# Autonomous-Drone-Racing-Lab/Efficient-Path-Planner

Measured on AMD Instinct MI355X. Metric: validity checks/sec + full plan ms/track, 1/2/4/8 MI355X vs CPU ref, higher is better.
Workload: dtype f64; 1 GPU; C2: 1 track, 8 gates, 64 OBBs, 1,048,576 sampled states per step; obbs=64, can_pass_gate=False, parallelism=replicas x1 (independent samplers), process_group=solo, launch=hip graph of the K steps

## Files before the change

### efficient-path-planner_amd/csrc/epp_internal.h

```cpp
#pragma once
#include <math.h>
#include <stdint.h>

#include <mutex>
#include <shared_mutex>
#include <string>
#include <vector>

#include <hip/hip_runtime_api.h>

#include "epp.h"

namespace epp {
epp_status generate_trajectory_into(const double* wp, int32_t n_wp, const double* times, double v_max,
                                    double a_max, double dt, double t0, const double v0[3], const double a0[3],
                                    double* (*alloc)(void*, int64_t), void* ctx, int64_t* n_rows);
struct FusedCheck {
    const epp_world* world;
    const double* xyz;
    int64_t n;
    double min_distance;
    uint8_t* valid;
};
epp_status check_and_generate_into(const FusedCheck* chk, const double* wp, int32_t n_wp, const double* times,
// ... 22 lines not shown
                                  const int64_t* rows_n, int32_t cap, int32_t k, int32_t can_pass_gate,
                                  uint8_t* valid, uint16_t* out16, int32_t target, int64_t* count, void* stream,
                                  const MotionMask* marks = nullptr);
bool knn_motions_rows_supported(const epp_world* world);

struct PlanSeg {
    uint64_t seed;
    double s[3], g[3];
    double bound;
    double gbound;
    double glo[3], ghi[3];
    double h;
    int64_t row_off;
    int64_t need_off;
    int32_t cap;
    int32_t need_cap;
};
enum : int { kPbRows = 1, kPbPerSeg = 3 };
struct PlanBatchLayout {
    int32_t S = 0, k = 0, ns_log = 0, nbc = 0, cap_total = 0, nctr = 0;
    int64_t ns = 0, NS = 0, need_cap = 0;
    size_t o_seg = 0, o_ctr = 0, o_xyz = 0, o_valid = 0, o_nodes = 0, o_cstat = 0, o_kws = 0, kws_stride = 0,
           o_query = 0, o_ids32 = 0, o_rows32 = 0, o_rows16 = 0, o_ev = 0, o_mark = 0, o_map = 0, o_nstat = 0,
           o_need = 0, dev_bytes = 0;
    size_t h_seg = 0, h_hdr = 0, h_slot = 0, h_rows = 0, h_need = 0, h_done = 0, host_bytes = 0;
    int32_t done_n = 0;
};
PlanBatchLayout plan_batch_layout(int32_t S, int64_t ns, int32_t k, PlanSeg* segs);
void plan_batch_trace_print();
epp_status plan_batch_launch(const epp_world* world, int32_t can_pass_gate, const double lo[3], const double hi[3],
                             const PlanBatchLayout& L, void* dev, void* host, uint32_t seq, void* stream);
}

namespace epp {

enum Field : int {
    F_LOX = 0, F_LOY, F_LOZ, F_HIX, F_HIY, F_HIZ,
    F_CX, F_CY, F_CZ,
    F_COS, F_SIN,
    F_HX, F_HY, F_HZ,
    EPP_NF
};

constexpr int kRecDoubles = 17;
constexpr int R_META = 16;

constexpr int kPtDoubles = 16;
constexpr int P_TX = F_HX, P_TY = F_HY, P_TZ = F_HZ;
#if defined(__HIPCC__)
__host__ __device__
#endif
constexpr uint32_t pt_chunk_off(uint32_t i, uint32_t c) { return (i << 7) + ((c ^ ((i >> 1) & 7u)) << 4); }
constexpr uint32_t kIdFill = 0x8000u;

constexpr size_t kListMaxLen = 4095;
constexpr size_t kStageBudget = 64 * 1024;

constexpr uint32_t META_FILLING = 1u;
constexpr uint32_t META_GATE = 2u;
constexpr int kMaxGridAxis = 255;

struct WorldView {
    const unsigned char* blob;
    uint32_t blob_bytes;
    int32_t n_obb;
    int32_t n_pad;
    int32_t nx, ny, nz;
    uint32_t front_bytes;
    uint32_t off_cell_mask;
    uint32_t off_cell_start;
    uint32_t off_cell_obb;
    uint32_t off_meta;
    uint32_t off_soa;
    double gx0, gy0, gz0;
    double gx1, gy1, gz1;
    double icx, icy, icz;
    float ofx, ofy, ofz;
    float i4x, i4y, i4z;
    float limx, limy, limz;
    float fmaxx, fmaxy, fmaxz;
    double r_gate, r_obst;
    uint32_t off_aos;
    uint32_t off_pt;
    uint32_t off_lists;
    uint32_t off_ids;
    uint32_t id_mask;
    uint32_t n_lists;
    uint32_t off_bitmap;
    uint32_t bm_words;
    uint32_t off_cls8;
    uint32_t cls8_bytes;
    int32_t bnx, bny, bnz;
    float bofx, bofy, bofz;
    float bix, biy, biz;
    uint32_t off_slab;
    int32_t slab_n;
    int32_t slab_log;
    int32_t slab_w;
    int32_t tile_n;
    uint32_t tile_words;
    float sofx, sofy, sofz;
    float six, siy, siz;
};

constexpr int kSlabMaxWords = 32;
constexpr size_t kSlabBudget = 40 * 1024;
constexpr size_t kSlabBudgetMax = 64 * 1024;
constexpr size_t kMotionsLdsFree = 150 * 1024 - 16 * (256 * 4 + 64);
#if defined(__HIPCC__)
__host__ __device__
#endif
constexpr int slab_row_stride(int w) { return (w & 1) ? w : w + 1; }

#if defined(__HIPCC__)
__host__ __device__
#endif
inline int slab_axis(double p, float off, float inv, int S) {
    float f = fmaf((float)p, inv, off);
    f = fminf(fmaxf(f, 0.0f), (float)(S - 1));
    return (int)f;
}

#if defined(__HIPCC__)
__host__ __device__
#endif
inline int bm_axis(double p, float off, float inv) {
    float f = fmaf((float)p, inv, off);
    f = fminf(fmaxf(f, -1.0f), 16777216.0f);
    return (int)f;
}

struct HostWorld {
    WorldView view{};
    std::vector<epp_obb> obbs;
    struct RecReader {
        hipStream_t stream;
        hipEvent_t ev;
        bool pending;
    };
    double* h_recs = nullptr;
    double* rec_buf[2] = {nullptr, nullptr};
    size_t rec_cap[2] = {0, 0};
    int rec_slot = 0;
    std::vector<RecReader> rec_readers[2];
    bool index_stale = false;
    std::mutex mu;
    std::shared_mutex index_mu;
    WorldView dev_view{};
    double r_gate = 0, r_obst = 0;
    int device = 0;
    void* d_blob = nullptr;
    const WorldView* d_view = nullptr;
    size_t d_capacity = 0;
    void* h_stage = nullptr;
    size_t h_capacity = 0;
    hipStream_t stream = nullptr;
    uint64_t generation = 0;
    std::string blob;
    std::vector<double> aabbs;
};

#if defined(__HIPCC__)
__host__ __device__
#endif
inline float fine_coord(double p, float o, float inv4) {
    return ((float)p - o) * inv4;
}
#if defined(__HIPCC__)
__host__ __device__
#endif
inline int fine_index(float f, int n) {
    const int nf = 4 * n;
    if (!(f >= 0.0f)) return 0;
    if (f >= (float)nf) return nf - 1;
    const int c = (int)f;
    return c < nf ? c : nf - 1;
}

void set_error(const std::string& msg);

struct SmallWorld {
    const double* recs;
    int32_t n_obb;
    double r_gate, r_obst;
    int host_slot;
    std::shared_lock<std::shared_mutex> lease;
};

struct IndexLease {
    std::shared_lock<std::shared_mutex> lk;
    WorldView view{};
    const WorldView* dview = nullptr;
};
epp_status ensure_index(const epp_world* w, IndexLease* lease = nullptr);

}
```

### efficient-path-planner_amd/csrc/states_v5.hip

```cpp
#include "states_diag.h"
#include "states_kernels.h"

namespace epp {
namespace {

constexpr int kStatesPerLane = 4;

struct WaveQueue5 {
    double x[64], y[64], z[64];
    uint32_t hdr[64];
};
template <int BLOCK>
constexpr uint32_t queue5_bytes() { return (BLOCK / 64) * sizeof(WaveQueue5); }

__device__ __forceinline__ uint32_t cell_axis5(double p, float off, float inv, uint32_t nm1) {
    const float f = fmaf((float)p, inv, off);
    int i;
    asm("v_cvt_i32_f32 %0, %1" : "=v"(i) : "v"(f));
    return min((uint32_t)i, nm1);
}
__device__ __forceinline__ uint32_t mad_u24(uint32_t a, uint32_t b, uint32_t c) {
    uint32_t r;
    asm("v_mad_u32_u24 %0, %1, %2, %3" : "=v"(r) : "v"(a), "s"(b), "v"(c));
    return r;
}
__device__ __forceinline__ uint32_t lane_scatter(uint32_t target, uint32_t data) {
    return (uint32_t)__builtin_amdgcn_ds_permute((int)((target & 63u) << 2), (int)data);
}

__device__ __forceinline__ bool point_rec_hit(const unsigned char* pts, uint32_t ide, double px, double py, double pz,
                                              bool can_pass) {
    typedef double f64x2 __attribute__((ext_vector_type(2)));
    const uint32_t i = ide & (kIdFill - 1u);
    f64x2 q[7];
#pragma unroll
    for (uint32_t k = 0; k < 7; ++k) q[k] = *reinterpret_cast<const f64x2*>(pts + pt_chunk_off(i, k));
    const double lox = q[0].x, loy = q[0].y, loz = q[1].x, hix = q[1].y, hiy = q[2].x, hiz = q[2].y;
    const double cx = q[3].x, cy = q[3].y, cz = q[4].x, c = q[4].y, s = q[5].x;
    const double tx = q[5].y, ty = q[6].x, tz = q[6].y;
    const bool in = (lox < px) & (px < hix) & (loy < py) & (py < hiy) & (loz < pz) & (pz < hiz);
    const bool skip = ((ide & kIdFill) != 0u) & can_pass;
    const double dx = px - cx, dy = py - cy, dz = pz - cz;
    const double lx = c * dx + s * dy;
    const double ly = c * dy - s * dx;
    return in & !skip & (fabs(lx) <= tx) & (fabs(ly) <= ty) & (fabs(dz) <= tz);
}

__device__ __forceinline__ bool states_exact_pt(const unsigned char* sbase, uint32_t lists_off, uint32_t ids_off,
                                                double px, double py, double pz, uint32_t cls, int can_pass) {
    const uint32_t h = reinterpret_cast<const uint32_t*>(sbase + lists_off)[cls];
    const uint16_t* ids = reinterpret_cast<const uint16_t*>(sbase + ids_off) + (h >> 12);
    const uint32_t cnt = h & 4095u;
    bool hit = false;
    for (uint32_t j = 0; j < cnt; ++j) hit |= point_rec_hit(sbase, ids[j], px, py, pz, can_pass != 0);
    return hit;
}

#ifdef EPP_STATES_TL
__device__ unsigned long long g_states_tl[kTlWaves][kTlWords];
#endif

struct V5Args {
    uint32_t lists_off, ids_off;
    uint32_t cls_off, cls_nz_off;
    uint32_t nx, ny, nz;
    float ox, oy, oz, ix, iy, iz;
};

template <bool MINDIST, bool COMPACT, int BLOCK, bool PREFETCH, bool C8, int SC>
__global__ __launch_bounds__(BLOCK) __attribute__((amdgpu_waves_per_eu(BLOCK == 512 && !PREFETCH ? 5 : BLOCK / 256)))
void k_states_v5(const unsigned char* stage_src, const double* xyz,
                                                     int64_t groups, uint32_t stage_bytes, int can_pass,
                                                     int64_t n, double md, uint8_t* __restrict__ valid,
                                                     int32_t* __restrict__ compact_idx,
                                                     unsigned long long* __restrict__ n_valid, V5Args wa) {
    __shared__ WaveQueue5 queues[BLOCK / 64];
    extern __shared__ __attribute__((aligned(16))) unsigned char lds_blob[];
    const int lane = threadIdx.x & 63;
    EPP_STL(0);
    WaveQueue5* qu = &queues[threadIdx.x >> 6];
    const int64_t stride = (int64_t)gridDim.x * BLOCK;
    const int64_t gfirst = (int64_t)blockIdx.x * BLOCK;
    int64_t g = gfirst + threadIdx.x;
    constexpr int NV = 3 * kStatesPerLane;
    double va[NV], vb[NV];
    const double* xyzb = groups > 0 ? xyz : reinterpret_cast<const double*>(stage_src);
    auto load = [&](int64_t grp, double (&dst)[NV]) {
        grp = grp < groups ? grp : groups - 1;
        grp = grp < 0 ? 0 : grp;
        const double2* q = reinterpret_cast<const double2*>(xyzb) + (NV / 2) * grp;
#pragma unroll
        for (int k = 0; k < NV / 2; ++k) {
            const double2 t = q[k];
            dst[2 * k] = t.x;
            dst[2 * k + 1] = t.y;
        }
    };
    typedef unsigned int u32x4 __attribute__((ext_vector_type(4)));
    constexpr int kStageChunks = SC;
    u32x4 stg[kStageChunks];
    const uint32_t n16 = stage_bytes / 16u;
#if defined(__HIP_DEVICE_COMPILE__)
    typedef const __attribute__((address_space(1))) u32x4* gptr_stage;
    const gptr_stage ssrc = (gptr_stage)stage_src;
#else
    const u32x4* ssrc = reinterpret_cast<const u32x4*>(stage_src);
#endif
#pragma unroll
    for (int i = 0; i < kStageChunks; ++i) {
        const uint32_t o = (uint32_t)(i * BLOCK) + threadIdx.x;
        stg[i] = ssrc[o < n16 ? o : n16 - 1u];
    }
    load(g, va);
#pragma unroll
    for (int i = 0; i < kStageChunks; ++i) {
        const uint32_t o = (uint32_t)(i * BLOCK) + threadIdx.x;
        *reinterpret_cast<u32x4*>(lds_blob + 16u * (o < n16 ? o : n16)) = stg[i];
    }
    const uint32_t lists_off = wa.lists_off, ids_off = wa.ids_off;
    const unsigned char* cls_base = lds_blob + wa.cls_off;
    [[maybe_unused]] const unsigned char* cls_nz = lds_blob + wa.cls_nz_off;
    const uint32_t* hdrs = reinterpret_cast<const uint32_t*>(lds_blob + lists_off);
    const uint16_t* ids_all = reinterpret_cast<const uint16_t*>(lds_blob + ids_off);
    const float ox = wa.ox, oy = wa.oy, oz = wa.oz, ix = wa.ix, iy = wa.iy, iz = wa.iz;
    const uint32_t nx = wa.nx, ny = wa.ny, nz = wa.nz;
    __syncthreads();
    EPP_STL(1);
    auto hit_of = [&](uint32_t ide, double px, double py, double pz) -> bool {
        if constexpr (MINDIST)
            return rec_hit<true>(reinterpret_cast<const double*>(lds_blob) + (size_t)(ide & (kIdFill - 1u)) * kRecDoubles,
                                 0.0, 0.0, px, py, pz, false, md);
        else
            return point_rec_hit(lds_blob, ide, px, py, pz, can_pass != 0);
    };
    auto cell_of = [&](double px, double py, double pz) -> uint32_t {
        const uint32_t cx = cell_axis5(px, ox, ix, nx - 1), cy = cell_axis5(py, oy, iy, ny - 1),
                       cz = cell_axis5(pz, oz, iz, nz - 1);
        return mad_u24(mad_u24(cz, ny, cy), nx, cx);
    };
    auto classes_of = [&](const auto& idx, auto& c, auto& occ) {
        constexpr int N = (int)(sizeof(idx) / sizeof(idx[0]));
        if (C8) {
            uint64_t wd[N];
            uint32_t rank[N];
#pragma unroll
            for (int k = 0; k < N; ++k) wd[k] = reinterpret_cast<const uint64_t*>(cls_base)[idx[k] >> 5];
#pragma unroll
            for (int k = 0; k < N; ++k) {
                const uint32_t m = (uint32_t)wd[k], sh = idx[k] & 31u;
                rank[k] = (uint32_t)(wd[k] >> 32) + (uint32_t)__popc(m & ((1u << sh) - 1u));
                occ[k] = (m >> sh) & 1u;
            }
#pragma unroll
            for (int k = 0; k < N; ++k) c[k] = (uint32_t)cls_nz[rank[k]];
#pragma unroll
            for (int k = 0; k < N; ++k) c[k] = occ[k] ? c[k] : 0u;
            return;
        }
#pragma unroll
        for (int k = 0; k < N; ++k) {
            c[k] = (uint32_t)reinterpret_cast<const uint16_t*>(cls_base)[idx[k]];
            occ[k] = c[k];
        }
    };
#ifdef EPP_STATES_TL
    uint32_t tl_needy = 0, tl_pairs = 0;
#endif
    auto process = [&](int64_t gg, const double (&v)[NV]) {
        const bool live = gg < groups;
        uint32_t c[kStatesPerLane];
        bool needy[kStatesPerLane];
        unsigned long long b[kStatesPerLane];
        uint32_t base[kStatesPerLane], total = 0;
#ifdef EPP_STATES_TL
        if (!PREFETCH) {
            asm volatile("s_waitcnt vmcnt(0)" ::: "memory");
            EPP_STL(2);
        }
#endif
        uint32_t cell[kStatesPerLane], occ[kStatesPerLane];
#pragma unroll
        for (int k = 0; k < kStatesPerLane; ++k) cell[k] = cell_of(v[3 * k], v[3 * k + 1], v[3 * k + 2]);
        classes_of(cell, c, occ);
        const uint32_t live_bits = live ? ~0u : 0u;
#pragma unroll
        for (int k = 0; k < kStatesPerLane; ++k) {
            needy[k] = (occ[k] & live_bits) != 0u;
            b[k] = __builtin_amdgcn_ballot_w64(needy[k]);
            base[k] = total;
            total += (uint32_t)__popcll(b[k]);
        }
        EPP_STL(3);
        uint32_t hd[kStatesPerLane];
#pragma unroll
        for (int k = 0; k < kStatesPerLane; ++k) hd[k] = hdrs[needy[k] ? c[k] : 0u];
        uint32_t hits = 0;
#ifdef EPP_STATES_NOEXACT
#pragma unroll
        for (int k = 0; k < kStatesPerLane; ++k) hits |= needy[k] ? 1u << k : 0u;
        if (false) {
#else
        if (total > 0) {
#endif
            uint32_t pos[kStatesPerLane];
#pragma unroll
            for (int k = 0; k < kStatesPerLane; ++k) pos[k] = base[k] + lanes_below(b[k]);
            for (uint32_t r0 = 0; r0 < total; r0 += 64) {
#pragma unroll
                for (int k = 0; k < kStatesPerLane; ++k) {
                    const uint32_t slot = pos[k] - r0;
                    if (needy[k] && slot < 64u) {
                        qu->x[slot] = v[3 * k];
                        qu->y[slot] = v[3 * k + 1];
                        qu->z[slot] = v[3 * k + 2];
                        qu->hdr[slot] = hd[k];
                    }
                }
                wave_lds_sync();
                const uint32_t tq = min(total - r0, 64u);
                const bool act = (uint32_t)lane < tq;
                const uint32_t hq = act ? qu->hdr[lane] : 0u;
                const uint32_t cnt = hq & 4095u, first = hq >> 12;
                uint32_t ptot;
                const uint32_t poff = wave_excl_scan(cnt, lane, ptot);
#ifdef EPP_STATES_TL
                tl_needy += tq;
                tl_pairs += ptot;
#endif
                bool hit_e = false;
                if (ptot <= 128u) {
                    uint32_t ln = (uint32_t)lane;
                    asm volatile("" : "+v"(ln));
                    const uint32_t head = (ln << 21) + (first - poff + ((1u << 21) + 128u));
                    const bool own0 = act & (poff < 64u);
                    const uint32_t head0 = (uint32_t)__builtin_amdgcn_readfirstlane((int)head);
                    const uint32_t h0 = dpp_incl_max(lane_scatter(own0 ? poff : 0u, own0 ? head : head0));
                    auto test = [&](uint32_t h, uint32_t q) {
                        const uint32_t e = (h >> 21) - 1u;
                        return q < ptot && hit_of(ids_all[(h & 0x1FFFFFu) + q - 128u], qu->x[e], qu->y[e], qu->z[e]);
                    };
                    unsigned long long m1 = 0ull;
                    uint32_t h1 = 0u;
                    if (ptot > 64u) {
                        const uint32_t plast = (uint32_t)__builtin_amdgcn_readlane((int)poff, (int)(tq - 1u));
                        const uint32_t hlast = (uint32_t)__builtin_amdgcn_readlane((int)head, (int)(tq - 1u));
                        const bool own1 = act & (poff >= 64u);
                        const uint32_t carry = (uint32_t)__builtin_amdgcn_readlane((int)h0, 63);
                        h1 = max(dpp_incl_max(lane_scatter(own1 ? poff : plast,
// ... 15 lines not shown
                    const double px = qu->x[lane], py = qu->y[lane], pz = qu->z[lane];
                    for (uint32_t j = 0; j < cnt; ++j) hit_e |= hit_of(idl[j], px, py, pz);
                }
                const unsigned long long hm = __builtin_amdgcn_ballot_w64(hit_e);
#pragma unroll
                for (int k = 0; k < kStatesPerLane; ++k) {
                    const uint32_t slot = pos[k] - r0;
                    if (needy[k] && slot < 64u && ((hm >> slot) & 1ull)) hits |= 1u << k;
                }
                wave_lds_sync();
            }
        }
        EPP_STL(4);
        const uint32_t fl = live ? (~hits & ((1u << kStatesPerLane) - 1u)) : 0u;
        if (live) *reinterpret_cast<uint32_t*>(valid + kStatesPerLane * gg) = pack_flags4(fl);
        if (COMPACT) compact_valid<kStatesPerLane>(fl, kStatesPerLane * gg, lane, compact_idx, n_valid);
    };
    if (PREFETCH) {
        for (int64_t g0 = gfirst; g0 < groups; g0 += 2 * stride, g += 2 * stride) {
            load(g + stride, vb);
            process(g, va);
            if (g0 + stride >= groups) break;
            load(g + 2 * stride, va);
            process(g + stride, vb);
        }
    } else {
        for (int64_t g0 = gfirst; g0 < groups; g0 += stride, g += stride) {
            if (g0 != gfirst) load(g, va);
            process(g, va);
        }
    }
#ifdef EPP_STATES_TL
    EPP_STL(5);
    if (lane == 0) {
        unsigned hw;
        asm volatile("s_getreg_b32 %0, hwreg(HW_REG_HW_ID)" : "=s"(hw));
        const int w_ = (int)((blockIdx.x * BLOCK + threadIdx.x) >> 6);
        if (w_ < kTlWaves)
            g_states_tl[w_][6] = hw | ((unsigned long long)min(tl_needy, 65535u) << 32) |
                                 ((unsigned long long)min(tl_pairs, 65535u) << 48);
    }
#endif
    if (blockIdx.x == 0 && threadIdx.x < (int)(n - kStatesPerLane * groups)) {
        const int64_t i = kStatesPerLane * groups + threadIdx.x;
        const double px = xyz[3 * i], py = xyz[3 * i + 1], pz = xyz[3 * i + 2];
        const uint32_t cell[1] = {cell_of(px, py, pz)};
        uint32_t c[1], occ[1];
        classes_of(cell, c, occ);
        bool hit = false;
        if (occ[0] != 0u) {
            if constexpr (MINDIST)
                hit = states_exact_rec<true>(lds_blob, lists_off, ids_off, kIdFill - 1u, 0.0, 0.0, px, py, pz, c[0], 0, md);
            else
                hit = states_exact_pt(lds_blob, lists_off, ids_off, px, py, pz, c[0], can_pass);
        }
        const bool ok = !hit;
        valid[i] = ok ? 1 : 0;
        if (COMPACT && ok) compact_idx[atomicAdd(n_valid, 1ull)] = (int32_t)i;
    }
}

uint32_t v5_start(const WorldView& w, bool mindist) { return mindist ? w.off_aos : w.off_pt; }
uint32_t v5_staged(const WorldView& w, bool mindist) {
    return (w.off_cls8 ? ((w.off_cls8 + w.cls8_bytes + 15u) & ~15u) : w.blob_bytes) - v5_start(w, mindist);
}
V5Args v5_args(const WorldView& w, bool mindist) {
    V5Args a{};
    const uint32_t start = v5_start(w, mindist);
    a.lists_off = w.off_lists - start;
    a.ids_off = w.off_ids - start;
    a.cls_off = (w.off_cls8 ? w.off_cls8 : w.off_bitmap) - start;
    a.cls_nz_off = a.cls_off + ((w.bm_words + 1u + 31u) >> 5) * 8u;
    a.nx = (uint32_t)w.bnx; a.ny = (uint32_t)w.bny; a.nz = (uint32_t)w.bnz;
    a.ox = w.bofx; a.oy = w.bofy; a.oz = w.bofz;
    a.ix = w.bix; a.iy = w.biy; a.iz = w.biz;
    return a;
}
constexpr uint32_t kV5DummyBytes = 96;
bool v5_fits(const WorldView& w, bool mindist) {
    const uint32_t sb = v5_staged(w, mindist);
    return sb <= kStageBudget && sb + 16u + queue5_bytes<1024>() <= 160u * 1024u && w.id_mask == kIdFill - 1u;
}

struct V5Shape {
    int64_t gN;
    int bs, grid;
    bool pf;
};
V5Shape v5_shape(int64_t n, uint32_t sb) {
    V5Shape r{};
    const int64_t cus = cu_count();
    r.gN = n / kStatesPerLane;
    const int forced = env_int("EPP_V5_BLOCK", 0);
    if (forced == 256 && 4u * (sb + 16u + queue5_bytes<256>()) <= 160u * 1024u && r.gN <= 4 * cus * 256) {
        r.bs = 256;
        r.grid = (int)std::max<int64_t>(1, (r.gN + 255) / 256);
        r.pf = false;
        return r;
    }
    const bool two = forced == 0 && 2u * (sb + 16u + queue5_bytes<512>()) <= 160u * 1024u && r.gN <= 2 * cus * 512;
    if (two) {
        r.bs = 512;
        r.grid = (int)std::max<int64_t>(1, (r.gN + 511) / 512);
        r.pf = false;
        return r;
    }
    const bool single = r.gN <= cus * 1024;
    r.bs = forced == 512 ? 512 : forced == 1024 ? 1024 : (single ? 1024 : 512);
    r.grid = (int)std::max<int64_t>(1, std::min<int64_t>((r.gN + r.bs - 1) / r.bs, cus));
    r.pf = r.gN > (int64_t)r.grid * r.bs;
    return r;
}

template <bool MINDIST>
void launch(const WorldView& w, const double* xyz, int64_t n, int32_t can_pass, double md, uint8_t* valid,
            int32_t* compact_idx, unsigned long long* nv, hipStream_t st) {
    const uint32_t sb = v5_staged(w, MINDIST);
    V5Shape sh = v5_shape(n, sb);
    if (sh.bs == 256 && compact_idx) {
        sh.bs = 512;
        sh.grid = (int)std::max<int64_t>(1, (sh.gN + 511) / 512);
    }
    const uint32_t dyn = sb + 16u;
    const unsigned char* src = w.blob + v5_start(w, MINDIST);
    const V5Args wa = v5_args(w, MINDIST);
#define EPP_LAUNCH_V5S(C, B, P, C8, SC)                                                                           \
    do {                                                                                                          \
        allow_lds(k_states_v5<MINDIST, C, B, P, C8, SC>, queue5_bytes<B>());                                      \
        hipLaunchKernelGGL((k_states_v5<MINDIST, C, B, P, C8, SC>), dim3(sh.grid), dim3(B), dyn, st, src, xyz,   \
                           sh.gN, sb, can_pass, n, md, valid, compact_idx, nv, wa);                               \
    } while (0)
    const bool half_stage = sb <= (uint32_t)kStageBudget / 2;
#define EPP_LAUNCH_V5C(C, B, P, C8)                                                              \
    do {                                                                                         \
        if (sb <= (uint32_t)B * 16u) EPP_LAUNCH_V5S(C, B, P, C8, 1);                              \
        else if (sb <= (uint32_t)B * 32u) EPP_LAUNCH_V5S(C, B, P, C8, 2);                         \
        else if (sb <= (uint32_t)B * 48u) EPP_LAUNCH_V5S(C, B, P, C8, 3);                         \
        else if (half_stage) EPP_LAUNCH_V5S(C, B, P, C8, (int)(kStageBudget / 2 / (B * 16)));    \
        else EPP_LAUNCH_V5S(C, B, P, C8, (int)(kStageBudget / (B * 16)));                        \
    } while (0)
#define EPP_LAUNCH_V5(C, B, P)                                 \
    do {                                                       \
        if (w.off_cls8) EPP_LAUNCH_V5C(C, B, P, true);          \
        else EPP_LAUNCH_V5C(C, B, P, false);                    \
    } while (0)
#define EPP_LAUNCH_V5B(B)                                \
    do {                                                 \
        if (sh.pf) {                                     \
            if (compact_idx) EPP_LAUNCH_V5(true, B, true);  \
            else EPP_LAUNCH_V5(false, B, true);          \
        } else {                                         \
            if (compact_idx) EPP_LAUNCH_V5(true, B, false); \
            else EPP_LAUNCH_V5(false, B, false);         \
        }                                                \
    } while (0)
    if (sh.bs == 256) EPP_LAUNCH_V5(false, 256, false);
    else if (sh.bs == 512) EPP_LAUNCH_V5B(512);
    else EPP_LAUNCH_V5B(1024);
#undef EPP_LAUNCH_V5B
#undef EPP_LAUNCH_V5
#undef EPP_LAUNCH_V5C
#undef EPP_LAUNCH_V5S
}

}

bool states_v5_fits(const WorldView& w, bool mindist, const double* xyz, int64_t n, const uint8_t* valid) {
    return v5_fits(w, mindist) && (reinterpret_cast<uintptr_t>(xyz) & 15) == 0 &&
           (reinterpret_cast<uintptr_t>(valid) & 3) == 0 &&
           (n >= kStatesPerLane || w.blob_bytes - v5_start(w, mindist) >= kV5DummyBytes);
}

epp_status launch_states_v5(const WorldView& w, bool mindist, const double* xyz, int64_t n, int32_t can_pass,
                            double md, uint8_t* valid, int32_t* compact_idx, int64_t* n_valid, hipStream_t st,
                            const char* what) {
    auto nv = reinterpret_cast<unsigned long long*>(n_valid);
    if (mindist) launch<true>(w, xyz, n, can_pass, md, valid, compact_idx, nv, st);
    else launch<false>(w, xyz, n, can_pass, md, valid, compact_idx, nv, st);
    return launch_error(what);
}

}

#ifdef EPP_STATES_TL
extern "C" epp_status epp_dbg_states_tl(unsigned long long* out, int64_t waves) {
    return hipMemcpyFromSymbol(out, HIP_SYMBOL(epp::g_states_tl),
                               (size_t)std::min<int64_t>(waves, epp::kTlWaves) * epp::kTlWords * 8) == hipSuccess
               ? EPP_OK
               : EPP_ERR_HIP;
}
#endif
```

### efficient-path-planner_amd/csrc/world_index.cpp

```cpp
#include <hip/hip_runtime.h>

#include <algorithm>
#include <chrono>
#include <cmath>
#include <cstdlib>
#include <cstring>
#include <mutex>
#include <new>
#include <string>
#include <vector>

#include "epp_internal.h"

namespace epp {
namespace {

void compute_aabb(const epp_obb& o, double inflate, double lo[3], double hi[3]) {
    static const double sx[8] = {-1, 1, 1, -1, -1, 1, 1, -1};
    static const double sy[8] = {-1, -1, 1, 1, -1, -1, 1, 1};
    static const double sz[8] = {-1, -1, -1, -1, 1, 1, 1, 1};
    for (int j = 0; j < 8; ++j) {
        const double c0 = sx[j] * o.half[0], c1 = sy[j] * o.half[1], c2 = sz[j] * o.half[2];
        for (int i = 0; i < 3; ++i) {
            const double g =
                ((o.rot[3 * i] * c0 + o.rot[3 * i + 1] * c1) + o.rot[3 * i + 2] * c2) + o.center[i];
            if (j == 0 || g < lo[i]) lo[i] = g;
            if (j == 0 || g > hi[i]) hi[i] = g;
        }
    }
    if (!o.filling) {
        for (int i = 0; i < 3; ++i) {
            lo[i] = lo[i] - inflate;
            hi[i] = hi[i] + inflate;
        }
    }
}

bool is_rz(const epp_obb& o) {
    const double* r = o.rot;
    return r[2] == 0.0 && r[5] == 0.0 && r[6] == 0.0 && r[7] == 0.0 && r[8] == 1.0 &&
           r[0] == r[4] && r[1] == -r[3];
}

inline size_t align16(size_t x) { return (x + 15) & ~size_t(15); }

bool build_records(HostWorld& hw, const epp_obb* obbs, int n) {
    for (int i = 0; i < n; ++i)
        if (!is_rz(obbs[i])) {
            set_error("epp_world: OBB rotation must be a rotation about z (src/Object.cpp:38-47)");
            return false;
        }
    const int slot = hw.h_recs ? 1 - hw.rec_slot : 0;
    for (auto& r : hw.rec_readers[slot])
        if (r.pending) {
            const hipError_t e = hipEventSynchronize(r.ev);
            if (e != hipSuccess) {
                set_error(std::string("epp_world: waiting for the readers of the records: ") + hipGetErrorString(e));
                return false;
            }
            r.pending = false;
        }
    const size_t need = std::max<size_t>(1, (size_t)n * kRecDoubles) * sizeof(double);
    if (need > hw.rec_cap[slot]) {
        if (hw.rec_buf[slot]) (void)hipHostFree(hw.rec_buf[slot]);
        hw.rec_buf[slot] = nullptr;
// ... 240 lines not shown
        }
        const size_t staged = align16((size_t)n * kRecDoubles * 8) + align16(hdr.size() * 4 + flat.size() * 2) +
                              align16(cls.size() * 2);
        if (staged > kStageBudget && target > 4096.0) {
            cls_target = target / 2;
            continue;
        }
        v.bnx = bd[0]; v.bny = bd[1]; v.bnz = bd[2];
        v.bofx = bo[0]; v.bofy = bo[1]; v.bofz = bo[2];
        v.bix = bi[0]; v.biy = bi[1]; v.biz = bi[2];
        v.bm_words = (uint32_t)cells;
        v.n_lists = (uint32_t)hdr.size();
        break;
    }
    const size_t n_entries = cell_start[ncell];
    const size_t off_mask = 0;
    const size_t off_cs = align16(off_mask + mask.size() * 8);
    const size_t front = align16(off_cs + cell_start.size() * 4);
    const size_t off_co = front;
    const size_t off_meta = align16(off_co + n_entries * 2);
    const size_t off_soa = align16(off_meta + meta.size() * 4);
    std::vector<double> aos((size_t)n * kRecDoubles, 0.0);
    for (int i = 0; i < n; ++i) {
        double* r = &aos[(size_t)i * kRecDoubles];
        const double* f = soa.data();
        const int fields[14] = {F_LOX, F_LOY, F_LOZ, F_HIX, F_HIY, F_HIZ, F_CX, F_CY, F_CZ, F_COS, F_SIN, F_HX, F_HY, F_HZ};
        for (int k = 0; k < 14; ++k) r[k] = f[(size_t)fields[k] * n_pad + i];
        uint64_t m = meta[i];
        std::memcpy(&r[R_META], &m, 8);
    }
    const bool id_flags = n <= 32768;
    std::vector<double> pts((size_t)n * kPtDoubles, 0.0);
    for (int i = 0; i < n; ++i) {
        const double* a = &aos[(size_t)i * kRecDoubles];
        const bool fill = (meta[i] & META_FILLING) != 0u;
        const double r = (meta[i] & META_GATE) ? hw.r_gate : hw.r_obst;
        double f[kPtDoubles] = {};
        for (int k = 0; k <= F_SIN; ++k) f[k] = a[k];
        const double ix = a[F_HX] + r, iy = a[F_HY] + r, iz = a[F_HZ] + r;
        f[P_TX] = fill ? a[F_HX] : ix;
        f[P_TY] = fill ? a[F_HY] : iy;
        f[P_TZ] = fill ? a[F_HZ] : iz;
        char* dst = reinterpret_cast<char*>(pts.data());
        for (uint32_t c = 0; c < 8; ++c) std::memcpy(dst + pt_chunk_off((uint32_t)i, c), &f[2 * c], 16);
    }
    if (id_flags)
        for (auto& id : flat) id = (uint16_t)(id | ((meta[id] & META_FILLING) ? kIdFill : 0u));
    const size_t off_aos = align16(off_soa + soa.size() * sizeof(double));
    const size_t off_pt = align16(off_aos + aos.size() * sizeof(double));
    const size_t off_lists = off_pt + pts.size() * sizeof(double);
    const size_t off_ids = off_lists + hdr.size() * 4;
    const bool c8 = hdr.size() <= 256;
    const size_t off_c8 = align16(off_ids + flat.size() * 2);
    std::vector<uint64_t> cwords;
    std::vector<uint8_t> cnz;
    if (c8) {
        cwords.assign((cls.size() + 31) / 32, 0ull);
        for (size_t w = 0; w < cwords.size(); ++w) {
            uint32_t m = 0;
            const uint64_t before = cnz.size();
            for (size_t j = 0; j < 32 && 32 * w + j < cls.size(); ++j)
                if (cls[32 * w + j]) {
                    m |= 1u << j;
                    cnz.push_back((uint8_t)cls[32 * w + j]);
                }
            cwords[w] = (uint64_t)m | (before << 32);
        }
    }
    const size_t c8_bytes = c8 ? cwords.size() * 8 + cnz.size() : 0;
    const size_t off_bm = c8 ? align16(off_c8 + c8_bytes) : off_c8;
    std::vector<uint32_t> slab;
    int S = 0, SL = 0, W = 0, T = 0;
    uint32_t tw = 0;
    float so[3] = {0, 0, 0}, si[3] = {0, 0, 0};
    std::vector<int> gsl((size_t)n * 6);
    const size_t slab_budget = std::max<size_t>(
        kSlabBudget, std::min<size_t>(kSlabBudgetMax, kMotionsLdsFree > (size_t)n * kRecDoubles * 8
                                                          ? kMotionsLdsFree - (size_t)n * kRecDoubles * 8
                                                          : 0));
    auto tile_words = [](int s_, int w_) {
        return (uint32_t)((6 * s_ * slab_row_stride(w_) + 3 * w_ + 16 * w_ + 3) & ~3);
    };
    auto place = [&](int t_, int sl_) {
        const int s_ = 1 << sl_;
        for (int k = 0; k < 3; ++k) {
            const int G = k < 2 ? t_ * s_ : s_;
            const double ext = std::max(g1[k] - g0[k], 1e-6);
            si[k] = (float)(G / ext);
            so[k] = (float)(-g0[k] * (G / ext));
            for (int i = 0; i < n; ++i) {
                const double* lo = &hw.aabbs[(size_t)i * 6];
                gsl[(size_t)i * 6 + k] = slab_axis(lo[k], so[k], si[k], G);
                gsl[(size_t)i * 6 + 3 + k] = slab_axis(lo[3 + k], so[k], si[k], G);
            }
        }
        std::vector<int> pop((size_t)t_ * t_, 0);
        for (int i = 0; i < n; ++i) {
            const int* g = &gsl[(size_t)i * 6];
            for (int ty = g[1] >> sl_; ty <= g[4] >> sl_; ++ty)
                for (int tx = g[0] >> sl_; tx <= g[3] >> sl_; ++tx) ++pop[(size_t)ty * t_ + tx];
        }
        return *std::max_element(pop.begin(), pop.end());
    };
    for (int min_sl = 4; n > 0 && !W && min_sl >= 2; min_sl -= 2)
        for (int w_ = 1; w_ <= kSlabMaxWords && !W; w_ *= 2)
            for (int t_ = 1; t_ <= 16 && !W; ++t_) {
                int sl_ = 6;
                while (sl_ >= min_sl && (size_t)t_ * t_ * tile_words(1 << sl_, w_) * 4 > slab_budget) --sl_;
                if (sl_ < min_sl) break;
                if (place(t_, sl_) <= 32 * w_) {
                    W = w_;
                    T = t_;
                    SL = sl_;
                }
            }
    if (W) {
        S = 1 << SL;
        place(T, SL);
        tw = tile_words(S, W);
        const int stride = slab_row_stride(W);
        slab.assign((size_t)T * T * tw, 0u);
        std::vector<int> fill_n((size_t)T * T, 0);
        for (int i = 0; i < n; ++i) {
            const int* g = &gsl[(size_t)i * 6];
            const int tx0 = g[0] >> SL, ty0 = g[1] >> SL;
            for (int ty = ty0; ty <= g[4] >> SL; ++ty)
                for (int tx = tx0; tx <= g[3] >> SL; ++tx) {
                    const size_t t = (size_t)ty * T + tx;
                    uint32_t* tile = &slab[t * tw];
                    const int j = fill_n[t]++;
                    const uint32_t bit = 1u << (j & 31);
                    const int wd = j >> 5;
                    const int l[3] = {std::min(std::max(g[0] - (tx << SL), 0), S - 1),
                                      std::min(std::max(g[1] - (ty << SL), 0), S - 1), g[2]};
                    const int h[3] = {std::min(std::max(g[3] - (tx << SL), 0), S - 1),
                                      std::min(std::max(g[4] - (ty << SL), 0), S - 1), g[5]};
                    for (int k = 0; k < 3; ++k) {
                        tile[((size_t)(2 * k) * S + l[k]) * stride + wd] |= bit;
                        tile[((size_t)(2 * k + 1) * S + h[k]) * stride + wd] |= bit;
                    }
                    uint32_t* tail = tile + (size_t)6 * S * stride;
                    if (tx == tx0) tail[wd] |= bit;
                    if (ty == ty0) tail[W + wd] |= bit;
                    if (meta[i] & META_FILLING) tail[2 * W + wd] |= bit;
                    reinterpret_cast<uint16_t*>(tail + 3 * W)[j] = (uint16_t)i;
                }
        }
        for (size_t t = 0; t < (size_t)T * T; ++t)
            for (int k = 0; k < 3; ++k) {
                uint32_t* le = &slab[t * tw + (size_t)(2 * k) * S * stride];
                uint32_t* ge = &slab[t * tw + (size_t)(2 * k + 1) * S * stride];
                for (int s_ = 1; s_ < S; ++s_)
                    for (int w_ = 0; w_ < W; ++w_) le[(size_t)s_ * stride + w_] |= le[(size_t)(s_ - 1) * stride + w_];
                for (int s_ = S - 2; s_ >= 0; --s_)
                    for (int w_ = 0; w_ < W; ++w_) ge[(size_t)s_ * stride + w_] |= ge[(size_t)(s_ + 1) * stride + w_];
            }
    }
    v.slab_n = S;
    v.slab_log = SL;
    v.slab_w = W;
    v.tile_n = T;
    v.tile_words = tw;
    v.sofx = so[0]; v.sofy = so[1]; v.sofz = so[2];
    v.six = si[0]; v.siy = si[1]; v.siz = si[2];
    const size_t off_slab = align16(off_bm + cls.size() * 2);
    const size_t total = align16(off_slab + slab.size() * 4);
    if (total > 0xFFFFFFFFull) {
        set_error("epp_world: index too large");
        return false;
    }
    hw.blob.assign(total, '\0');
    char* b = &hw.blob[0];
    std::memcpy(b + off_mask, mask.data(), mask.size() * 8);
    std::memcpy(b + off_cs, cell_start.data(), cell_start.size() * 4);
    if (n_entries) std::memcpy(b + off_co, cell_obb.data(), n_entries * 2);
    std::memcpy(b + off_meta, meta.data(), meta.size() * 4);
    std::memcpy(b + off_soa, soa.data(), soa.size() * sizeof(double));
    if (!aos.empty()) std::memcpy(b + off_aos, aos.data(), aos.size() * sizeof(double));
    if (!pts.empty()) std::memcpy(b + off_pt, pts.data(), pts.size() * sizeof(double));
    std::memcpy(b + off_lists, hdr.data(), hdr.size() * 4);
    if (!flat.empty()) std::memcpy(b + off_ids, flat.data(), flat.size() * 2);
    v.off_ids = (uint32_t)off_ids;
    v.id_mask = id_flags ? kIdFill - 1u : 0xFFFFu;
    v.off_aos = (uint32_t)off_aos;
    v.off_pt = (uint32_t)off_pt;
    std::memcpy(b + off_bm, cls.data(), cls.size() * 2);
    if (!slab.empty()) std::memcpy(b + off_slab, slab.data(), slab.size() * 4);
    v.off_slab = (uint32_t)off_slab;
    if (c8) {
        std::memcpy(b + off_c8, cwords.data(), cwords.size() * 8);
        if (!cnz.empty()) std::memcpy(b + off_c8 + cwords.size() * 8, cnz.data(), cnz.size());
    }
    v.off_cls8 = c8 ? (uint32_t)off_c8 : 0u;
    v.cls8_bytes = (uint32_t)c8_bytes;
    v.off_lists = (uint32_t)off_lists;
    v.off_bitmap = (uint32_t)off_bm;
    v.blob_bytes = (uint32_t)total;
    v.front_bytes = (uint32_t)front;
    v.off_cell_mask = (uint32_t)off_mask;
    v.off_cell_start = (uint32_t)off_cs;
    v.off_cell_obb = (uint32_t)off_co;
    v.off_meta = (uint32_t)off_meta;
    v.off_soa = (uint32_t)off_soa;
    return true;
}

bool upload(HostWorld& hw) {
    const size_t bytes = hw.blob.size();
    const size_t view_off = (bytes + 255) & ~size_t(255);
    const size_t need = view_off + sizeof(WorldView);
    hipError_t e = hipSuccess;
    if (!hw.stream) e = hipStreamCreateWithFlags(&hw.stream, hipStreamNonBlocking);
    if (e == hipSuccess && need > hw.d_capacity) {
        if (hw.d_blob) (void)hipFree(hw.d_blob);
        hw.d_blob = nullptr;
        hw.d_capacity = 0;
        e = hipMalloc(&hw.d_blob, need);
        if (e == hipSuccess) hw.d_capacity = need;
    }
    if (e == hipSuccess && need > hw.h_capacity) {
        if (hw.h_stage) (void)hipHostFree(hw.h_stage);
        hw.h_stage = nullptr;
        hw.h_capacity = 0;
        e = hipHostMalloc(&hw.h_stage, need, hipHostMallocDefault);
        if (e == hipSuccess) hw.h_capacity = need;
    }
    if (e != hipSuccess) {
        set_error(std::string("epp_world: allocation: ") + hipGetErrorString(e));
        return false;
    }
    hw.view.blob = (const unsigned char*)hw.d_blob;
    hw.d_view = reinterpret_cast<const WorldView*>(static_cast<char*>(hw.d_blob) + view_off);
    hw.dev_view = hw.view;
    std::memcpy(hw.h_stage, hw.blob.data(), bytes);
    std::memcpy(static_cast<char*>(hw.h_stage) + view_off, &hw.view, sizeof(WorldView));
    e = hipMemcpyAsync(hw.d_blob, hw.h_stage, need, hipMemcpyHostToDevice, hw.stream);
    if (e == hipSuccess) e = hipStreamSynchronize(hw.stream);
    if (e != hipSuccess) {
        set_error(std::string("epp_world: upload: ") + hipGetErrorString(e));
        return false;
    }
    return true;
}

struct WorldBufs {
    int device = 0;
    double* rec_buf[2] = {nullptr, nullptr};
// ... 219 lines not shown
    }
    if (e == hipSuccess) e = hipEventRecord(r->ev, st);
    if (e != hipSuccess) {
        set_error(std::string("epp_world: recording a reader of the records: ") + hipGetErrorString(e));
        return EPP_ERR_HIP;
    }
    r->pending = true;
    return EPP_OK;
}

}

extern "C" epp_status epp_dbg_world_info(const epp_world* w, int64_t out[6]) {
    if (!w || !out) return EPP_ERR_INVALID_ARGUMENT;
    const epp::WorldView& v = w->view;
    out[0] = v.blob_bytes;
    out[1] = v.off_bitmap;
    out[2] = v.n_lists;
    out[3] = (int64_t)v.bnx * v.bny * v.bnz;
    out[4] = (int64_t)v.nx * v.ny * v.nz;
    out[5] = v.n_obb;
    return EPP_OK;
}

extern "C" epp_status epp_dbg_build_blob(const epp_obb* obbs, int32_t n, double r_gate, double r_obst, int32_t reps,
                                         double out[6]) {
    if (!out || n < 0 || (n > 0 && !obbs) || reps < 1) return EPP_ERR_INVALID_ARGUMENT;
    epp::HostWorld hw;
    hw.r_gate = r_gate;
    hw.r_obst = r_obst;
    const auto t0 = std::chrono::steady_clock::now();
    for (int r = 0; r < reps; ++r)
        if (!epp::build_blob(hw, obbs, n)) return EPP_ERR_UNSUPPORTED;
    const auto t1 = std::chrono::steady_clock::now();
    out[0] = std::chrono::duration<double, std::micro>(t1 - t0).count() / reps;
    out[1] = hw.view.blob_bytes;
    out[2] = hw.view.tile_n;
    out[3] = hw.view.tile_words;
    out[4] = hw.view.slab_w;
    out[5] = hw.view.slab_n;
    return EPP_OK;
}

extern "C" epp_status epp_dbg_class_layout(const epp_obb* obbs, int32_t n, double r_gate, double r_obst,
                                           int64_t out[12]) {
    if (!out || n < 0 || (n > 0 && !obbs)) return EPP_ERR_INVALID_ARGUMENT;
    epp::HostWorld hw;
    hw.r_gate = r_gate;
    hw.r_obst = r_obst;
    if (!epp::build_blob(hw, obbs, n)) return EPP_ERR_UNSUPPORTED;
    const epp::WorldView& v = hw.view;
    const int64_t vals[12] = {v.off_aos, v.off_lists, v.off_ids, v.off_cls8, v.off_bitmap, v.blob_bytes, v.n_lists,
                              v.bm_words, v.bnx, v.bny, v.bnz,
                              (int64_t)((v.off_cls8 ? ((v.off_cls8 + v.cls8_bytes + 15u) & ~15u) : v.blob_bytes) -
                                        v.off_pt)};
    for (int k = 0; k < 12; ++k) out[k] = vals[k];
    return EPP_OK;
}

extern "C" epp_status epp_dbg_point_records(const epp_obb* obbs, int32_t n, double r_gate, double r_obst,
                                            double* recs17, double* pt16, uint16_t* ids, int64_t ids_cap,
                                            int64_t out[6]) {
    if (!out || n < 0 || (n > 0 && (!obbs || !recs17 || !pt16)) || ids_cap < 0 || (ids_cap > 0 && !ids))
        return EPP_ERR_INVALID_ARGUMENT;
    epp::HostWorld hw;
    hw.r_gate = r_gate;
    hw.r_obst = r_obst;
    if (!epp::build_blob(hw, obbs, n)) return EPP_ERR_UNSUPPORTED;
    const epp::WorldView& v = hw.view;
    const char* b = hw.blob.data();
    int64_t n_ids = 0;
    for (uint32_t l = 0; l < v.n_lists; ++l) {
        uint32_t h;
        std::memcpy(&h, b + v.off_lists + 4 * (size_t)l, 4);
        n_ids = std::max<int64_t>(n_ids, (int64_t)(h >> 12) + (h & 4095u));
    }
    if (n > 0) std::memcpy(recs17, b + v.off_aos, (size_t)n * epp::kRecDoubles * 8);
    for (int i = 0; i < n; ++i)
        for (uint32_t c = 0; c < 8; ++c)
            std::memcpy(pt16 + (size_t)i * epp::kPtDoubles + 2 * c, b + v.off_pt + epp::pt_chunk_off((uint32_t)i, c), 16);
    if (ids_cap > 0) std::memcpy(ids, b + v.off_ids, (size_t)std::min<int64_t>(ids_cap, n_ids) * 2);
    const int64_t vals[6] = {v.off_aos, v.off_pt, v.off_lists, v.off_ids, n_ids, v.id_mask};
    for (int k = 0; k < 6; ++k) out[k] = vals[k];
    return EPP_OK;
}

extern "C" int64_t epp_dbg_check_sparse_classes(const epp_obb* obbs, int32_t n, double r_gate, double r_obst) {
    if (n < 0 || (n > 0 && !obbs)) return -2;
    epp::HostWorld hw;
    hw.r_gate = r_gate;
    hw.r_obst = r_obst;
    if (!epp::build_blob(hw, obbs, n)) return -2;
    const epp::WorldView& v = hw.view;
    if (!v.off_cls8) return -1;
    const unsigned char* b = reinterpret_cast<const unsigned char*>(hw.blob.data());
    const uint16_t* cls = reinterpret_cast<const uint16_t*>(b + v.off_bitmap);
    const unsigned char* base = b + v.off_cls8;
    const unsigned char* nz = base + ((v.bm_words + 1u + 31u) >> 5) * 8u;
    int64_t bad = 0;
    for (uint32_t idx = 0; idx <= v.bm_words; ++idx) {
        uint64_t wd;
        std::memcpy(&wd, base + (size_t)(idx >> 5) * 8, 8);
        const uint32_t m = (uint32_t)wd, sh = idx & 31u;
        const uint32_t rank = (uint32_t)(wd >> 32) + (uint32_t)__builtin_popcount(m & ((1u << sh) - 1u));
        const uint32_t c = ((m >> sh) & 1u) ? (uint32_t)nz[rank] : 0u;
        bad += c != (uint32_t)cls[idx];
    }
    return bad;
}
// ... 1 lines not shown
```

Baseline: 152.5 billion state validity checks/s.

## Add cell-header image to states kernel, storing list headers and prebaked record addresses

Builds an alternate compact LDS image for the plain (non-min-distance) state check. In it, the compressed class bitmap maps directly to 32-bit list headers, and the id lists store pre-swizzled record byte offsets with a gate flag in the low bit. The kernel gets a new CLS template mode that skips the class-byte to header indirection and the per-record chunk-offset arithmetic. The image is built by default only when it stages in no more chunks than the existing layout, which may add blob size and template instantiations.

New measurement: 151.7 billion state validity checks/s. No clear change (-0.5%).

```diff
diff --git a/efficient-path-planner_amd/csrc/epp_internal.h b/efficient-path-planner_amd/csrc/epp_internal.h
--- a/efficient-path-planner_amd/csrc/epp_internal.h
+++ b/efficient-path-planner_amd/csrc/epp_internal.h
@@ -98,6 +98,9 @@
 #endif
 constexpr uint32_t pt_chunk_off(uint32_t i, uint32_t c) { return (i << 7) + ((c ^ ((i >> 1) & 7u)) << 4); }
 constexpr uint32_t kIdFill = 0x8000u;
+
+constexpr uint32_t kHidFill = 1u;
+constexpr int kHimgMaxObbs = 512;
 
 constexpr size_t kListMaxLen = 4095;
 constexpr size_t kStageBudget = 64 * 1024;
@@ -136,6 +139,10 @@
     uint32_t bm_words;
     uint32_t off_cls8;
     uint32_t cls8_bytes;
+    uint32_t off_himg;
+    uint32_t off_hcls;
+    uint32_t off_hids;
+    uint32_t himg_bytes;
     int32_t bnx, bny, bnz;
     float bofx, bofy, bofz;
     float bix, biy, biz;
@@ -203,6 +210,7 @@
     hipStream_t stream = nullptr;
     uint64_t generation = 0;
     std::string blob;
+    int himg_mode = -1;
     std::vector<double> aabbs;
 };
 
diff --git a/efficient-path-planner_amd/csrc/states_v5.hip b/efficient-path-planner_amd/csrc/states_v5.hip
--- a/efficient-path-planner_amd/csrc/states_v5.hip
+++ b/efficient-path-planner_amd/csrc/states_v5.hip
@@ -28,33 +28,37 @@
     return (uint32_t)__builtin_amdgcn_ds_permute((int)((target & 63u) << 2), (int)data);
 }
 
+template <bool ADDR>
 __device__ __forceinline__ bool point_rec_hit(const unsigned char* pts, uint32_t ide, double px, double py, double pz,
                                               bool can_pass) {
     typedef double f64x2 __attribute__((ext_vector_type(2)));
-    const uint32_t i = ide & (kIdFill - 1u);
+    const uint32_t i = ide & (kIdFill - 1u), a0 = ide & ~kHidFill;
     f64x2 q[7];
 #pragma unroll
-    for (uint32_t k = 0; k < 7; ++k) q[k] = *reinterpret_cast<const f64x2*>(pts + pt_chunk_off(i, k));
+    for (uint32_t k = 0; k < 7; ++k)
+        q[k] = *reinterpret_cast<const f64x2*>(pts + (ADDR ? a0 ^ (k << 4) : pt_chunk_off(i, k)));
     const double lox = q[0].x, loy = q[0].y, loz = q[1].x, hix = q[1].y, hiy = q[2].x, hiz = q[2].y;
     const double cx = q[3].x, cy = q[3].y, cz = q[4].x, c = q[4].y, s = q[5].x;
     const double tx = q[5].y, ty = q[6].x, tz = q[6].y;
     const bool in = (lox < px) & (px < hix) & (loy < py) & (py < hiy) & (loz < pz) & (pz < hiz);
-    const bool skip = ((ide & kIdFill) != 0u) & can_pass;
+    const bool skip = ((ide & (ADDR ? kHidFill : kIdFill)) != 0u) & can_pass;
     const double dx = px - cx, dy = py - cy, dz = pz - cz;
     const double lx = c * dx + s * dy;
     const double ly = c * dy - s * dx;
     return in & !skip & (fabs(lx) <= tx) & (fabs(ly) <= ty) & (fabs(dz) <= tz);
 }
 
-__device__ __forceinline__ bool states_exact_pt(const unsigned char* sbase, uint32_t lists_off, uint32_t ids_off,
-                                                double px, double py, double pz, uint32_t cls, int can_pass) {
-    const uint32_t h = reinterpret_cast<const uint32_t*>(sbase + lists_off)[cls];
+template <bool ADDR>
+__device__ __forceinline__ bool states_exact_pt(const unsigned char* sbase, uint32_t h, uint32_t ids_off, double px,
+                                                double py, double pz, int can_pass) {
     const uint16_t* ids = reinterpret_cast<const uint16_t*>(sbase + ids_off) + (h >> 12);
     const uint32_t cnt = h & 4095u;
     bool hit = false;
-    for (uint32_t j = 0; j < cnt; ++j) hit |= point_rec_hit(sbase, ids[j], px, py, pz, can_pass != 0);
+    for (uint32_t j = 0; j < cnt; ++j) hit |= point_rec_hit<ADDR>(sbase, ids[j], px, py, pz, can_pass != 0);
     return hit;
 }
+
+enum : int { kClsU16 = 0, kClsBytes = 1, kClsHeaders = 2 };
 
 #ifdef EPP_STATES_TL
 __device__ unsigned long long g_states_tl[kTlWaves][kTlWords];
@@ -67,7 +71,7 @@
     float ox, oy, oz, ix, iy, iz;
 };
 
-template <bool MINDIST, bool COMPACT, int BLOCK, bool PREFETCH, bool C8, int SC>
+template <bool MINDIST, bool COMPACT, int BLOCK, bool PREFETCH, int CLS, int SC>
 __global__ __launch_bounds__(BLOCK) __attribute__((amdgpu_waves_per_eu(BLOCK == 512 && !PREFETCH ? 5 : BLOCK / 256)))
 void k_states_v5(const unsigned char* stage_src, const double* xyz,
                                                      int64_t groups, uint32_t stage_bytes, int can_pass,
@@ -118,9 +122,11 @@
         *reinterpret_cast<u32x4*>(lds_blob + 16u * (o < n16 ? o : n16)) = stg[i];
     }
     const uint32_t lists_off = wa.lists_off, ids_off = wa.ids_off;
+    static_assert(CLS != kClsHeaders || !MINDIST, "the header image is the plain test's");
+    constexpr bool HDR = CLS == kClsHeaders;
     const unsigned char* cls_base = lds_blob + wa.cls_off;
     [[maybe_unused]] const unsigned char* cls_nz = lds_blob + wa.cls_nz_off;
-    const uint32_t* hdrs = reinterpret_cast<const uint32_t*>(lds_blob + lists_off);
+    [[maybe_unused]] const uint32_t* hdrs = reinterpret_cast<const uint32_t*>(lds_blob + lists_off);
     const uint16_t* ids_all = reinterpret_cast<const uint16_t*>(lds_blob + ids_off);
     const float ox = wa.ox, oy = wa.oy, oz = wa.oz, ix = wa.ix, iy = wa.iy, iz = wa.iz;
     const uint32_t nx = wa.nx, ny = wa.ny, nz = wa.nz;
@@ -131,7 +137,7 @@
             return rec_hit<true>(reinterpret_cast<const double*>(lds_blob) + (size_t)(ide & (kIdFill - 1u)) * kRecDoubles,
                                  0.0, 0.0, px, py, pz, false, md);
         else
-            return point_rec_hit(lds_blob, ide, px, py, pz, can_pass != 0);
+            return point_rec_hit<HDR>(lds_blob, ide, px, py, pz, can_pass != 0);
     };
     auto cell_of = [&](double px, double py, double pz) -> uint32_t {
         const uint32_t cx = cell_axis5(px, ox, ix, nx - 1), cy = cell_axis5(py, oy, iy, ny - 1),
@@ -140,7 +146,7 @@
     };
     auto classes_of = [&](const auto& idx, auto& c, auto& occ) {
         constexpr int N = (int)(sizeof(idx) / sizeof(idx[0]));
-        if (C8) {
+        if (CLS != kClsU16) {
             uint64_t wd[N];
             uint32_t rank[N];
 #pragma unroll
@@ -150,6 +156,11 @@
                 const uint32_t m = (uint32_t)wd[k], sh = idx[k] & 31u;
                 rank[k] = (uint32_t)(wd[k] >> 32) + (uint32_t)__popc(m & ((1u << sh) - 1u));
                 occ[k] = (m >> sh) & 1u;
+            }
+            if (HDR) {
+#pragma unroll
+                for (int k = 0; k < N; ++k) c[k] = reinterpret_cast<const uint32_t*>(cls_nz)[rank[k]];
+                return;
             }
 #pragma unroll
             for (int k = 0; k < N; ++k) c[k] = (uint32_t)cls_nz[rank[k]];
@@ -193,7 +204,7 @@
         EPP_STL(3);
         uint32_t hd[kStatesPerLane];
 #pragma unroll
-        for (int k = 0; k < kStatesPerLane; ++k) hd[k] = hdrs[needy[k] ? c[k] : 0u];
+        for (int k = 0; k < kStatesPerLane; ++k) hd[k] = HDR ? c[k] : hdrs[needy[k] ? c[k] : 0u];
         uint32_t hits = 0;
 #ifdef EPP_STATES_NOEXACT
 #pragma unroll
@@ -315,7 +326,7 @@
             if constexpr (MINDIST)
                 hit = states_exact_rec<true>(lds_blob, lists_off, ids_off, kIdFill - 1u, 0.0, 0.0, px, py, pz, c[0], 0, md);
             else
-                hit = states_exact_pt(lds_blob, lists_off, ids_off, px, py, pz, c[0], can_pass);
+                hit = states_exact_pt<HDR>(lds_blob, HDR ? c[0] : hdrs[c[0]], ids_off, px, py, pz, can_pass);
         }
         const bool ok = !hit;
         valid[i] = ok ? 1 : 0;
@@ -323,16 +334,26 @@
     }
 }
 
-uint32_t v5_start(const WorldView& w, bool mindist) { return mindist ? w.off_aos : w.off_pt; }
+bool v5_himg(const WorldView& w, bool mindist) { return !mindist && w.off_himg != 0u; }
+uint32_t v5_start(const WorldView& w, bool mindist) {
+    return v5_himg(w, mindist) ? w.off_himg : mindist ? w.off_aos : w.off_pt;
+}
 uint32_t v5_staged(const WorldView& w, bool mindist) {
-    return (w.off_cls8 ? ((w.off_cls8 + w.cls8_bytes + 15u) & ~15u) : w.blob_bytes) - v5_start(w, mindist);
+    if (v5_himg(w, mindist)) return w.himg_bytes;
+    const uint32_t end = w.off_himg ? w.off_himg : w.blob_bytes;
+    return (w.off_cls8 ? ((w.off_cls8 + w.cls8_bytes + 15u) & ~15u) : end) - v5_start(w, mindist);
 }
 V5Args v5_args(const WorldView& w, bool mindist) {
     V5Args a{};
     const uint32_t start = v5_start(w, mindist);
-    a.lists_off = w.off_lists - start;
-    a.ids_off = w.off_ids - start;
-    a.cls_off = (w.off_cls8 ? w.off_cls8 : w.off_bitmap) - start;
+    if (v5_himg(w, mindist)) {
+        a.ids_off = w.off_hids - start;
+        a.cls_off = w.off_hcls - start;
+    } else {
+        a.lists_off = w.off_lists - start;
+        a.ids_off = w.off_ids - start;
+        a.cls_off = (w.off_cls8 ? w.off_cls8 : w.off_bitmap) - start;
+    }
     a.cls_nz_off = a.cls_off + ((w.bm_words + 1u + 31u) >> 5) * 8u;
     a.nx = (uint32_t)w.bnx; a.ny = (uint32_t)w.bny; a.nz = (uint32_t)w.bnz;
     a.ox = w.bofx; a.oy = w.bofy; a.oz = w.bofz;
@@ -387,25 +408,31 @@
     const uint32_t dyn = sb + 16u;
     const unsigned char* src = w.blob + v5_start(w, MINDIST);
     const V5Args wa = v5_args(w, MINDIST);
-#define EPP_LAUNCH_V5S(C, B, P, C8, SC)                                                                           \
+#define EPP_LAUNCH_V5S(C, B, P, CLS, SC)                                                                          \
     do {                                                                                                          \
-        allow_lds(k_states_v5<MINDIST, C, B, P, C8, SC>, queue5_bytes<B>());                                      \
-        hipLaunchKernelGGL((k_states_v5<MINDIST, C, B, P, C8, SC>), dim3(sh.grid), dim3(B), dyn, st, src, xyz,   \
+        allow_lds(k_states_v5<MINDIST, C, B, P, CLS, SC>, queue5_bytes<B>());                                      \
+        hipLaunchKernelGGL((k_states_v5<MINDIST, C, B, P, CLS, SC>), dim3(sh.grid), dim3(B), dyn, st, src, xyz,   \
                            sh.gN, sb, can_pass, n, md, valid, compact_idx, nv, wa);                               \
     } while (0)
     const bool half_stage = sb <= (uint32_t)kStageBudget / 2;
-#define EPP_LAUNCH_V5C(C, B, P, C8)                                                              \
+#define EPP_LAUNCH_V5C(C, B, P, CLS)                                                             \
     do {                                                                                         \
-        if (sb <= (uint32_t)B * 16u) EPP_LAUNCH_V5S(C, B, P, C8, 1);                              \
-        else if (sb <= (uint32_t)B * 32u) EPP_LAUNCH_V5S(C, B, P, C8, 2);                         \
-        else if (sb <= (uint32_t)B * 48u) EPP_LAUNCH_V5S(C, B, P, C8, 3);                         \
-        else if (half_stage) EPP_LAUNCH_V5S(C, B, P, C8, (int)(kStageBudget / 2 / (B * 16)));    \
-        else EPP_LAUNCH_V5S(C, B, P, C8, (int)(kStageBudget / (B * 16)));                        \
+        if (sb <= (uint32_t)B * 16u) EPP_LAUNCH_V5S(C, B, P, CLS, 1);                              \
+        else if (sb <= (uint32_t)B * 32u) EPP_LAUNCH_V5S(C, B, P, CLS, 2);                         \
+        else if (sb <= (uint32_t)B * 48u) EPP_LAUNCH_V5S(C, B, P, CLS, 3);                         \
+        else if (half_stage) EPP_LAUNCH_V5S(C, B, P, CLS, (int)(kStageBudget / 2 / (B * 16)));    \
+        else EPP_LAUNCH_V5S(C, B, P, CLS, (int)(kStageBudget / (B * 16)));                        \
     } while (0)
 #define EPP_LAUNCH_V5(C, B, P)                                 \
     do {                                                       \
-        if (w.off_cls8) EPP_LAUNCH_V5C(C, B, P, true);          \
-        else EPP_LAUNCH_V5C(C, B, P, false);                    \
+        if constexpr (!MINDIST) {                               \
+            if (w.off_himg) {                                   \
+                EPP_LAUNCH_V5C(C, B, P, kClsHeaders);           \
+                break;                                          \
+            }                                                   \
+        }                                                       \
+        if (w.off_cls8) EPP_LAUNCH_V5C(C, B, P, kClsBytes);     \
+        else EPP_LAUNCH_V5C(C, B, P, kClsU16);                  \
     } while (0)
 #define EPP_LAUNCH_V5B(B)                                \
     do {                                                 \
diff --git a/efficient-path-planner_amd/csrc/world_index.cpp b/efficient-path-planner_amd/csrc/world_index.cpp
--- a/efficient-path-planner_amd/csrc/world_index.cpp
+++ b/efficient-path-planner_amd/csrc/world_index.cpp
@@ -11,6 +11,7 @@
 #include <vector>
 
 #include "epp_internal.h"
+#include "launch_helpers.h"
 
 namespace epp {
 namespace {
@@ -357,23 +358,39 @@
     const size_t off_ids = off_lists + hdr.size() * 4;
     const bool c8 = hdr.size() <= 256;
     const size_t off_c8 = align16(off_ids + flat.size() * 2);
+    const int himg_mode = hw.himg_mode >= 0 ? hw.himg_mode : env_int("EPP_V5_CELL_HEADERS", -1);
+    const bool himg_can = n > 0 && n <= kHimgMaxObbs && id_flags && (himg_mode > 0 || (himg_mode < 0 && c8));
     std::vector<uint64_t> cwords;
     std::vector<uint8_t> cnz;
-    if (c8) {
+    std::vector<uint32_t> chdr;
+    if (c8 || himg_can) {
         cwords.assign((cls.size() + 31) / 32, 0ull);
         for (size_t w = 0; w < cwords.size(); ++w) {
             uint32_t m = 0;
-            const uint64_t before = cnz.size();
+            const uint64_t before = chdr.size();
             for (size_t j = 0; j < 32 && 32 * w + j < cls.size(); ++j)
                 if (cls[32 * w + j]) {
                     m |= 1u << j;
-                    cnz.push_back((uint8_t)cls[32 * w + j]);
+                    if (c8) cnz.push_back((uint8_t)cls[32 * w + j]);
+                    chdr.push_back(hdr[cls[32 * w + j]]);
                 }
             cwords[w] = (uint64_t)m | (before << 32);
         }
     }
     const size_t c8_bytes = c8 ? cwords.size() * 8 + cnz.size() : 0;
     const size_t off_bm = c8 ? align16(off_c8 + c8_bytes) : off_c8;
+    const size_t himg_bytes =
+        align16(pts.size() * sizeof(double) + cwords.size() * 8 + chdr.size() * 4 + flat.size() * 2);
+    const size_t plain_bytes = align16(off_c8 + c8_bytes) - off_pt;
+    constexpr size_t kChunk = 512 * 16;
+    const bool himg = himg_can && (himg_mode == 2 || (himg_mode == 1 && himg_bytes <= kStageBudget) ||
+                                   (himg_mode < 0 && (himg_bytes + kChunk - 1) / kChunk <= (plain_bytes + kChunk - 1) / kChunk));
+    std::vector<uint16_t> hids;
+    if (himg) {
+        hids.resize(flat.size());
+        for (size_t j = 0; j < flat.size(); ++j)
+            hids[j] = (uint16_t)(pt_chunk_off(flat[j] & (kIdFill - 1u), 0) | ((flat[j] & kIdFill) ? kHidFill : 0u));
+    }
     std::vector<uint32_t> slab;
     int S = 0, SL = 0, W = 0, T = 0;
     uint32_t tw = 0;
@@ -469,7 +486,10 @@
     v.sofx = so[0]; v.sofy = so[1]; v.sofz = so[2];
     v.six = si[0]; v.siy = si[1]; v.siz = si[2];
     const size_t off_slab = align16(off_bm + cls.size() * 2);
-    const size_t total = align16(off_slab + slab.size() * 4);
+    const size_t off_himg = align16(off_slab + slab.size() * 4);
+    const size_t off_hcls = off_himg + pts.size() * sizeof(double);
+    const size_t off_hids = off_hcls + cwords.size() * 8 + chdr.size() * 4;
+    const size_t total = off_himg + (himg ? himg_bytes : 0);
     if (total > 0xFFFFFFFFull) {
         set_error("epp_world: index too large");
         return false;
@@ -498,6 +518,16 @@
     }
     v.off_cls8 = c8 ? (uint32_t)off_c8 : 0u;
     v.cls8_bytes = (uint32_t)c8_bytes;
+    if (himg) {
+        std::memcpy(b + off_himg, pts.data(), pts.size() * sizeof(double));
+        std::memcpy(b + off_hcls, cwords.data(), cwords.size() * 8);
+        if (!chdr.empty()) std::memcpy(b + off_hcls + cwords.size() * 8, chdr.data(), chdr.size() * 4);
+        if (!hids.empty()) std::memcpy(b + off_hids, hids.data(), hids.size() * 2);
+    }
+    v.off_himg = himg ? (uint32_t)off_himg : 0u;
+    v.off_hcls = himg ? (uint32_t)off_hcls : 0u;
+    v.off_hids = himg ? (uint32_t)off_hids : 0u;
+    v.himg_bytes = himg ? (uint32_t)himg_bytes : 0u;
     v.off_lists = (uint32_t)off_lists;
     v.off_bitmap = (uint32_t)off_bm;
     v.blob_bytes = (uint32_t)total;
@@ -823,9 +853,28 @@
     const epp::WorldView& v = hw.view;
     const int64_t vals[12] = {v.off_aos, v.off_lists, v.off_ids, v.off_cls8, v.off_bitmap, v.blob_bytes, v.n_lists,
                               v.bm_words, v.bnx, v.bny, v.bnz,
-                              (int64_t)((v.off_cls8 ? ((v.off_cls8 + v.cls8_bytes + 15u) & ~15u) : v.blob_bytes) -
-                                        v.off_pt)};
+                              v.off_himg ? (int64_t)v.himg_bytes
+                                         : (int64_t)((v.off_cls8 ? ((v.off_cls8 + v.cls8_bytes + 15u) & ~15u) : v.blob_bytes) -
+                                                     v.off_pt)};
     for (int k = 0; k < 12; ++k) out[k] = vals[k];
+    return EPP_OK;
+}
+
+extern "C" epp_status epp_dbg_header_image(const epp_obb* obbs, int32_t n, double r_gate, double r_obst, int32_t mode,
+                                           unsigned char* buf, int64_t cap, int64_t out[16]) {
+    if (!out || n < 0 || (n > 0 && !obbs) || cap < 0 || (cap > 0 && !buf)) return EPP_ERR_INVALID_ARGUMENT;
+    epp::HostWorld hw;
+    hw.r_gate = r_gate;
+    hw.r_obst = r_obst;
+    hw.himg_mode = mode;
+    if (!epp::build_blob(hw, obbs, n)) return EPP_ERR_UNSUPPORTED;
+    const epp::WorldView& v = hw.view;
+    if ((int64_t)hw.blob.size() <= cap) std::memcpy(buf, hw.blob.data(), hw.blob.size());
+    const uint32_t old_end = v.off_cls8 ? ((v.off_cls8 + v.cls8_bytes + 15u) & ~15u) : (v.off_himg ? v.off_himg : v.blob_bytes);
+    const int64_t vals[16] = {v.blob_bytes, v.off_pt, v.off_lists, v.off_ids, v.off_bitmap, v.bm_words, v.n_lists,
+                              v.off_cls8, v.cls8_bytes, v.off_himg, v.off_hcls, v.off_hids, v.himg_bytes, v.n_obb,
+                              v.id_mask, (int64_t)old_end - v.off_pt};
+    for (int k = 0; k < 16; ++k) out[k] = vals[k];
     return EPP_OK;
 }
 
```
